# uguryagmur/RealTimeObjectDetection

Hardware: AMD Instinct MI355X
Metric: frames/sec YOLOv3 608x608 bs=8 (Darknet.forward + write_results; 2 batches in flight, write_results_async on a second stream) (higher is better)
Workload: dtype f16x2-split (3 MFMA products, f32 accumulate); 1 GPU; YOLOv3 cfg 608x608 batch=8 per GPU, split-f16 MFMA conv + fused head + GPU NMS (BASELINE configs[2]); precision=f16s3, tiles=autotune (this run), parallelism=frame-shard x1, in_flight_batches=2, detections_last_step=1699, candidates_last_step=1914, f16_range_overflow=False

## Files before the change

realtimeobjectdetection_amd/csrc/conv_bandd_common.h:

```cpp
#pragma once
#include "conv_f16s3_common.h"

namespace rtod {

#ifdef RTOD_TIMELINE
constexpr int BD_EPI_BLOCKS = 2048;
static __device__ unsigned long long g_bandd_epi[BD_EPI_BLOCKS * 5];
#define BD_ESTAMP(slot) { const unsigned long long tn_ = __builtin_amdgcn_s_memtime(); et_[slot] += tn_ - eprev_; eprev_ = tn_; }
#else
#define BD_ESTAMP(slot)
#endif

template <int NBASE, int PER = 2> __device__ __forceinline__ void bandd_wait_vmcnt_plus(int n) {
    static_assert(((NBASE == 4 || NBASE == 8) && PER == 2) || ((NBASE == 2 || NBASE == 4) && PER == 1), "two B sets of 1, 2 or 4 loads");
    asm volatile("" : "+s"(n));
    if (n == 0) vmcnt<NBASE>();
    else if (n == 1) vmcnt<NBASE + PER>();
    else if (n == 2) vmcnt<NBASE + 2 * PER>();
    else if (n == 3) vmcnt<NBASE + 3 * PER>();
    else if (n == 4) vmcnt<NBASE + 4 * PER>();
    else vmcnt<NBASE + 5 * PER>();
}

template <int BM, int BN, int WM, int WN, int NT, int RG, bool RES, int KG, bool F16 = false, bool RAW = false>
__device__ __forceinline__ void bandd_epilogue(const ConvArgs& a, f32x4 (&acc)[WM / 16][WN / 16], unsigned char* smem, int bm, int bn, int tid,
                                               int wm, int wn, int lr, int lh, int M, int kg) {
    constexpr int TM = WM / 16, TN = WN / 16, MT = 16, TS = BN;
    static_assert(BM % RG == 0 && RG % 16 == 0, "epilogue pass");
    static_assert(!RAW || (!RES && !F16), "raw-sum instances: no shortcut, no plain-f16 store");
#ifdef RTOD_TIMELINE
    unsigned long long et_[5] = {0, 0, 0, 0, 0};
    unsigned long long eprev_ = __builtin_amdgcn_s_memtime();
#endif
    float* T = reinterpret_cast<float*>(smem);
    float amax = 0.f;
    const float escale = RAW ? 1.0f : SPLIT_SCALE;
    constexpr int GPR = BN / 8;
// ... 91 lines not shown
```

realtimeobjectdetection_amd/csrc/conv_bandd_f16s3.hip:

```cpp
#include "conv_bandd_common.h"
#include <cstdio>
#include <cstdlib>
#include <map>
#include <vector>
#include <algorithm>

namespace rtod {

constexpr int BANDD_MAX_W = 94;
constexpr int BANDD_WIDE_W = 160;

#ifdef RTOD_TIMELINE
constexpr int BD_TL_BLOCKS = 2048, BD_TL_N = 8;
__device__ unsigned long long g_bandd_tl[BD_TL_BLOCKS * BD_TL_N];
#define BD_STAMP(slot) { const unsigned long long tn_ = __builtin_amdgcn_s_memtime(); tl_[slot] += tn_ - tl_prev_; tl_prev_ = tn_; }
#else
#define BD_STAMP(slot)
#endif
__host__ __device__ constexpr int bandd_rows(int bm, int w) { return (bm + 2 * w + 2 + 15) / 16 * 16; }

template <int BM, int BN, int NWM, int NWN, int MINW, int EPI, int BUFM, int KG, int MAXW>
__global__ __launch_bounds__(NWM * NWN * 64 * KG, MINW)
void conv_bandd_f16s3_kernel(const ConvArgs a, const int grid_m, const int grid_n) {
    constexpr bool F16 = epi_f16(EPI);
// ... 295 lines not shown
                    fprintf(stderr, "[timeline]   wg duration us min %.1f p10 %.1f p50 %.1f p90 %.1f max %.1f | end us p10 %.1f p50 %.1f p90 %.1f max %.1f | CUs seen %d, with 1/2/3/4/5 wgs: %d %d %d %d %d\n",
                            dur[0], dur[nb / 10], dur[nb / 2], dur[nb * 9 / 10], dur[nb - 1], en[nb / 10], en[nb / 2], en[nb * 9 / 10], en[nb - 1],
                            (int)per_cu.size(), hist[1], hist[2], hist[3], hist[4], hist[5]);
                    double ss[16] = {0}, sd[16] = {0}; int sn[16] = {0};
                    for (int b = 0; b < nb; ++b) { const int tg = (int)((h[b * BD_TL_N + 2] >> 16) & 15); ++sn[tg]; ss[tg] += (h[b * BD_TL_N] - t0) / 100.0; sd[tg] += (h[b * BD_TL_N + 1] - h[b * BD_TL_N]) / 100.0; }
                    for (int tg = 0; tg < 16; ++tg) if (sn[tg]) fprintf(stderr, "[timeline]   slot %d: %d wgs, mean start %.1f us, mean duration %.1f us\n", tg, sn[tg], ss[tg] / sn[tg], sd[tg] / sn[tg]);
                }
                ++printed;
            }
        }
    }
#endif
    return hip_fail(hipGetLastError(), "conv_bandd_f16s3 launch");
}

#define RTOD_BANDD_TILES(X) \
    X(0, 128, 128, 1, 4, 3, 0, 1, 94, "") X(1, 128, 128, 1, 4, 3, 1, 1, 94, ",db") X(2, 64, 128, 1, 4, 4, 1, 1, 94, ",db") \
    X(3, 64, 128, 1, 4, 4, 1, 2, 94, ",db,k2") X(4, 128, 128, 1, 4, 2, 1, 2, 94, ",db,k2") \
    X(5, 96, 128, 1, 4, 3, 1, 1, 94, ",db") X(6, 96, 128, 1, 4, 3, 1, 2, 94, ",db,k2") \
    X(7, 128, 128, 1, 4, 2, 0, 1, 160, ",w160") X(8, 48, 128, 1, 4, 3, 1, 2, 94, ",db,k2")

#define RTOD_X_INFO(idx, bm, bn, nwm, nwn, minw, db, kg, maxw, sfx) {bm, bn, "conv_bandd_f16s3<" #bm "x" #bn "," #nwm "x" #nwn sfx ">"},
static const ConvVariantInfo kBanddModes[BANDD_MODES] = { RTOD_BANDD_TILES(RTOD_X_INFO) };
#undef RTOD_X_INFO
const ConvVariantInfo& conv_bandd_mode_info(int idx) { return kBanddModes[idx < 0 || idx >= BANDD_MODES ? 0 : idx]; }
bool conv_bandd_wide_supported(int ksize, int stride, int pad, int cin, int w_in) {
    return ksize == 3 && stride == 1 && pad == 1 && cin % 32 == 0 && w_in > BANDD_MAX_W && w_in <= BANDD_WIDE_W;
}
int conv_bandd_mode_kg(int idx) {
#define RTOD_X_KG(i, bm, bn, nwm, nwn, minw, db, kg, maxw, sfx) if (idx == i) return kg;
// ... 31 lines not shown
```

realtimeobjectdetection_amd/csrc/plan.h:

```cpp
#pragma once
#include <functional>
#include <map>
#include <string>
#include <vector>

#include "rtod_internal.h"

namespace rtod {

enum LayerType { LT_CONV = 0, LT_SHORTCUT, LT_ROUTE, LT_UPSAMPLE, LT_MAXPOOL, LT_YOLO };
const char* layer_type_name(int t);

struct Layer {
    int index = 0;
    int type = LT_CONV;
    int cin = 0, cout = 0, hin = 0, win = 0, hout = 0, wout = 0;
    int size = 0, stride = 1, pad = 0;
    bool bn = false;
    int act = 0;
    bool nearest = false;
    bool decode_v5 = false;
    int pool_pad = 0;
    std::vector<int> srcs;
    std::vector<std::pair<int, int>> anchors;
// ... 92 lines not shown
    bool opt_patch_kernel = true;
    bool opt_ring_kernel = true;
    bool opt_pwd_kernel = true;
    bool opt_fuse_shortcut = true;
    bool opt_fuse_decode = true;
    bool opt_zero_copy_concat = true;
    bool opt_narrow_cin = false;
    bool opt_stem_pool = false;
    bool opt_keep_head_inputs = false;
    bool opt_keep_block_inputs = false;
    bool opt_keep_neck_activations = false;
    bool opt_keep_backbone_activations = false;
    bool opt_fuse_stem_pool = true;
    int opt_force_f16s3_variant = -1;
    int opt_force_f32_variant = -1;
    int32_t* overflow_flag = nullptr;
    std::vector<hipEvent_t> events;

    ~Plan();
    int parse(const std::string& cfg_text);
    int resolve_shapes();
    int plan_buffers();
    DecodeArgs decode_args(const Layer& yolo) const;
    int replan_or(const std::function<void()>& restore);
    void assign_arena();
    void layout_weights();
    bool uses_split(const Layer& L) const;
    int check_split_supported(int mode) const;
    int pack_weights(const float* w, size_t n, std::vector<float>& packed) const;
    void pack_conv(const PackedConv& pc, const float* p, float* blk) const;
// ... 80 lines not shown
```

realtimeobjectdetection_amd/csrc/plan_build.cpp:

```cpp
#include "plan.h"

#include <algorithm>
#include <cstdarg>
#include <sstream>

namespace rtod {

static thread_local std::string g_err;

void set_error(const char* fmt, ...) {
    char buf[1024];
    va_list ap;
    va_start(ap, fmt);
    vsnprintf(buf, sizeof(buf), fmt, ap);
    va_end(ap);
    g_err = buf;
}
const std::string& last_error_string() { return g_err; }

int hip_fail(hipError_t e, const char* what) {
    if (e == hipSuccess) return RTOD_OK;
    set_error("HIP error %d (%s) at %s", (int)e, hipGetErrorString(e), what);
    return RTOD_E_HIP;
}
// ... 32 lines not shown
        {"fuse_pointwise", &Plan::opt_fuse_pointwise}, {"ring_kernel", &Plan::opt_ring_kernel}, {"pwd_kernel", &Plan::opt_pwd_kernel},
        {"stem2_kernel", &Plan::opt_stem2_kernel}, {"k_slices", &Plan::opt_k_slices}, {"bn_batch_stats", &Plan::opt_bn_batch_stats},
        {"bn_batch_split", &Plan::opt_bn_batch_split}, {"bn_split_narrow", &Plan::opt_bn_split_narrow}, {"fuse_bn_pool", &Plan::opt_fuse_bn_pool},
        {"k_slice_workgroups", &Plan::opt_k_slice_workgroups}, {"k_slices_split", &Plan::opt_k_slices_split}, {"patch_kernel", &Plan::opt_patch_kernel},
        {"stem_kernel", &Plan::opt_stem_kernel}, {"band_kernel", &Plan::opt_band_kernel}, {"fuse_shortcut", &Plan::opt_fuse_shortcut},
        {"fuse_decode", &Plan::opt_fuse_decode}, {"zero_copy_concat", &Plan::opt_zero_copy_concat}, {"narrow_cin", &Plan::opt_narrow_cin},
        {"stem_pool", &Plan::opt_stem_pool}, {"fuse_stem_pool", &Plan::opt_fuse_stem_pool}, {"keep_head_inputs", &Plan::opt_keep_head_inputs},
        {"keep_block_inputs", &Plan::opt_keep_block_inputs}, {"keep_neck_activations", &Plan::opt_keep_neck_activations},
        {"keep_backbone_activations", &Plan::opt_keep_backbone_activations},
    };
    const std::string k(name);
    bool* flag = nullptr; int* num = nullptr;
    for (const auto& f : kFlags) if (k == f.name) flag = &(this->*f.flag);
    if (k == "force_f16s3_variant") num = &opt_force_f16s3_variant;
    else if (k == "force_f32_variant") num = &opt_force_f32_variant;
    else if (!flag) { set_error("set_option: unknown option '%s'", name); return RTOD_E_ARG; }
    if (flag == &opt_bn_batch_stats && value && height != width) { set_error("set_option: bn_batch_stats is not supported on a rectangular plan (%dx%d)", height, width); return RTOD_E_ARG; }
    const bool old_flag = flag ? *flag : false; const int old_num = num ? *num : 0;
    if (flag) *flag = value != 0; else *num = value;
    return replan_or([&] { if (flag) *flag = old_flag; else *num = old_num; });
}

int Plan::replan_or(const std::function<void()>& restore) {
    reset_planning();
    int rc = plan_buffers();
    if (!rc && precision >= 1) rc = check_split_supported(precision);
    if (rc) {
        const std::string msg = last_error_string();
        restore();
        reset_planning();
// ... 459 lines not shown
```

realtimeobjectdetection_amd/csrc/plan_forward.cpp:

```cpp
#include "plan.h"

#include <algorithm>
#include <cstring>

namespace rtod {

bool Plan::pw_active() const { return precision == 1 && opt_fuse_pointwise && !bn_split_active(); }
bool Plan::stem2_active() const { return precision == 1 && !bn_split_active() && opt_stem2_kernel && stem2_pattern && !keep_all && convs[launches[0].conv_slot].split; }
bool Plan::fusions_held() const { return opt_keep_backbone_activations; }
int Plan::fused_pool(int layer) const {
    if (keep_all) return -1;
    if (layer == 0 && precision >= 1 && stem_pool_pattern && convs[launches[0].conv_slot].stem16) return 1;
    return bn_narrow_active() && opt_fuse_bn_pool ? layers[layer].bn_pool : -1;
}

LaunchForm Plan::form(size_t li) const {
    LaunchForm f;
    const Launch& l = launches[li];
    switch (l.kind) {
        case LK_MAXPOOL:
            if (li > 0 && launches[li - 1].conv_slot >= 0 && fused_pool(launches[li - 1].layer) == l.layer) f.inside = (int)li - 1;
            return f;
        case LK_STEM: if (stem2_active()) f.inside = 1; break;
        case LK_CONV:
// ... 24 lines not shown
    const View in = view_of(l.in_layer);
    a.in = in.base; a.in_ldc = in.ldc; a.in_coff = in.coff;
    a.B = batch; a.Hi = L.hin; a.Wi = L.win; a.Cin = pc.cin_p;
    a.w = d_weights + pc.w_off; a.bias = d_weights + pc.b_off; a.K = pc.K; a.Kpad = pc.Kpad; a.Npad = pc.Npad;
    a.in_bytes = (unsigned)std::min<int64_t>((int64_t)batch * in.H * in.W * in.ldc * 4, 0xFFFFFFFFll);
    a.w_bytes = (unsigned)std::min<int64_t>((int64_t)pc.Npad * pc.Kpad * 2, 0xFFFFFFFFll);
    if (pc.split) {
        a.w_hi = reinterpret_cast<const _Float16*>(d_weights + pc.w_off);
        a.w_lo = reinterpret_cast<const _Float16*>(d_weights + pc.wl_off);
        a.inv_scale = d_weights + pc.s_off;
        a.f16 = precision == 2 ? 1 : 0;
    }
    a.kh = a.kw = L.size; a.stride = L.stride; a.pad = L.pad;
    a.Ho = L.hout; a.Wo = L.wout; a.Cout = L.cout; a.leaky = L.act;
    a.ovf = overflow_flag;
    if (in.C != pc.cin_p || in.H != L.hin || in.W != L.win) { set_error("forward: layer %d input view mismatch", l.layer); return RTOD_E_STATE; }
    if (l.out_layer == -2) { a.out = out; a.dec = l.dec; a.dec.train = train_decode; }
    else {
        const View o = view_of(l.out_layer);
        if (!o.base || o.C != L.cout || o.H != L.hout || o.W != L.wout) { set_error("forward: layer %d output view mismatch", l.layer); return RTOD_E_STATE; }
        a.out = o.base; a.out_ldc = o.ldc; a.out_coff = o.coff; a.out_split = o.split;
    }
    if (l.in2_layer >= 0) {
        const View r = view_of(l.in2_layer);
        if (!r.base || r.C != L.cout || r.H != L.hout || r.W != L.wout) { set_error("forward: layer %d residual view mismatch", l.layer); return RTOD_E_STATE; }
        a.res = r.base; a.res_ldc = r.ldc; a.res_coff = r.coff;
    }
    if (f.guest >= 0) {
        const Launch& g = launches[f.guest];
        const Layer& G = layers[g.layer];
// ... 215 lines not shown
```

realtimeobjectdetection_amd/csrc/plan_tiles.cpp:

```cpp
#include "plan.h"

#include <algorithm>
#include <mutex>

namespace rtod {

int Plan::choose_variant(const Layer& L, int batch) const {
    if (opt_force_f32_variant >= 0 && opt_force_f32_variant < CV_COUNT) return opt_force_f32_variant;
    if (L.cout <= 32) return CV_128x32;
    if (L.cout <= 64) return CV_128x64;
    const int64_t M = (int64_t)batch * L.hout * L.wout;
    const int64_t big = ((M + 127) / 128) * ((L.cout + 127) / 128);
    return big >= 512 ? CV_128x128 : CV_64x64;
}

int Plan::f32_slice_mode(const Launch& l, int batch, int variant) const {
    const PackedConv& pc = convs[l.conv_slot];
    if (pc.split || pc.stem || pc.slice_chunks <= 0) return 0;
    const Layer& L = layers[l.layer];
    const ConvVariantInfo& vi = conv_variant_info(variant);
    const int64_t M = (int64_t)batch * L.hout * L.wout;
    const int64_t tiles = ((M + vi.bm - 1) / vi.bm) * ((L.cout + vi.bn - 1) / vi.bn);
    const int64_t S = (pc.Kpad / 32 + pc.slice_chunks - 1) / pc.slice_chunks;
    return (opt_k_slice_workgroups && d_scratch && tiles < 512 && S * M * pc.Npad <= scratch_floats) ? 2 : 1;
}

bool Plan::tile_legal(const Launch& l, int v) const {
    const TileRef t = family_of(v);
    if (!t || l.kind != LK_CONV || l.conv_slot < 0 || !convs[l.conv_slot].split) return false;
    const PackedConv& pc = convs[l.conv_slot];
    const Layer& L = layers[l.layer];
    if (precision == 2 && !t.f16()) return false;
    if (raw_launch(l) && !t.raw()) return false;
    if (pc.narrow || t.is(TF_C16)) return pc.narrow && t.is(TF_C16);
    if (pc.ks_chunks > 0 || t.is(TF_KS)) return pc.ks_chunks > 0 && t.is(TF_KS);
    if (pc.band) return t.is(TF_BAND) && conv_band_mode_valid(t.mode, L.cin, L.hin, L.win);
    const bool hosts_pw = form(&l - &launches[0]).guest >= 0, plain = l.out_layer != -2 && !hosts_pw, same_map = L.hout == L.hin && L.wout == L.win;
    switch (t.fam->id) {
        case TF_GENERIC: return !(hosts_pw && t.fam->info(t.mode).bn < L.cout);
        case TF_BAND: return t.bandd_wide() && opt_band_kernel && plain && same_map && pc.Npad % 128 == 0 && pc.K == pc.Kpad &&
                             conv_bandd_wide_supported(L.size, L.stride, L.pad, pc.cin_p, L.win);
        case TF_RING: return !hosts_pw && L.act <= 1;
        case TF_PWD: return opt_pwd_kernel && plain && same_map && conv_pwd_supported(L.size, L.stride, L.pad, pc.cin_p);
        case TF_PATCH: return plain && L.act <= 1 && L.hout == L.hin && conv_patch_supported(L.size, L.stride, L.pad, L.cin, L.cout) &&
                              conv_patch_mode_valid(t.mode, L.cin, L.cout);
    }
    return false;
}

int Plan::default_tile(const Launch& l, int batch) const {
    const PackedConv& pc = convs[l.conv_slot];
// ... 13 lines not shown
}

int Plan::variant_for(const Launch& l, int batch) const {
    int want = opt_force_f16s3_variant;
    if (want < 0) {
        auto it = tuned.find(batch);
        const size_t idx = &l - &launches[0];
        if (it != tuned.end() && idx < it->second.size()) want = it->second[idx];
    }
    int v = want >= 0 && tile_legal(l, want) ? want : default_tile(l, batch);
    if (family_of(v).ks_sched_b() && !(opt_k_slice_workgroups && ks_sched_b_fits(l, batch))) --v;
    return v;
}

std::vector<int> Plan::tile_candidates(const Launch& l, int batch) const {
    static const int kOrder[TF_COUNT] = {TF_GENERIC, TF_PATCH, TF_BAND, TF_PWD, TF_RING, TF_C16, TF_KS};
    const int cout = layers[l.layer].cout;
    const bool ks_b = opt_k_slice_workgroups && ks_sched_b_fits(l, batch);
    std::vector<int> cand;
    for (int f : kOrder) {
        if ((f == TF_RING && !opt_ring_kernel) || (f == TF_PATCH && !opt_patch_kernel)) continue;
        const TileFamily& F = tile_family(f);
        for (int m = 0; m < F.modes; ++m) {
            const int bn = F.info(m).bn;
            const bool too_wide = f == TF_GENERIC || f == TF_RING ? bn > 64 && bn > 2 * ((cout + 63) / 64 * 64)
                                : f == TF_PATCH ? bn > 64 && bn > cout
                                : f == TF_PWD ? bn > 128 && bn > (cout + 127) / 128 * 128 : false;
            if (too_wide || (family_of(F.base + m).ks_sched_b() && !ks_b) || !tile_legal(l, F.base + m)) continue;
            cand.push_back(F.base + m);
        }
    }
// ... 1 lines not shown
}

int Plan::launch_split_variant(ConvArgs& a, const PackedConv& pc, int v, hipStream_t s) const {
    const TileRef t = family_of(v);
    if (!t) { set_error("variant %d is no split-f16 tile", v); return RTOD_E_STATE; }
    if (precision == 2 && !t.f16()) { set_error("variant %d has no plain-f16 instance", v); return RTOD_E_STATE; }
    if (a.raw_out && !t.raw()) { set_error("variant %d has no raw-sum instance", v); return RTOD_E_STATE; }
    if (pc.narrow != t.is(TF_C16)) {
        set_error(pc.narrow ? "variant %d requested for a narrow (Cin = 16) layer" : "narrow variant %d requested for a layer without tap-major weights", v);
        return RTOD_E_STATE;
    }
    if ((pc.ks_chunks > 0) != t.is(TF_KS)) {
        set_error(pc.ks_chunks > 0 ? "variant %d requested for a K-sliced layer" : "K-sliced variant %d requested for a layer that is not sliced", v);
        return RTOD_E_STATE;
    }
    if (pc.band != t.is(TF_BAND) && !(t.bandd_wide() && !pc.band)) {
        set_error(pc.band ? "variant %d requested for a band layer" : "band variant %d requested for a layer without band weights", v);
        return RTOD_E_STATE;
    }
    if (t.is(TF_KS)) {
        a.slice_chunks = pc.ks_chunks;
        a.partial = nullptr; a.partial_floats = 0;
        if (t.ks_sched_b()) { a.partial = d_scratch; a.partial_floats = scratch_floats; }
    }
    return t.fam->launch(a, t.mode, s);
}

static std::mutex g_tune_mutex;
static std::map<std::vector<int>, int> g_tune_memo;

int Plan::tune_launch(size_t li, ConvArgs& a, int batch, hipStream_t s) {
// ... 87 lines not shown
```

realtimeobjectdetection_amd/csrc/rtod_internal.h:

```cpp
#pragma once
#include <hip/hip_runtime.h>
#if defined(RTOD_STAMPS) && !defined(RTOD_DIAG)
#define RTOD_DIAG 1
#endif
#include <algorithm>
#include <atomic>
#include <cstdint>
#include <cstdio>
#include <string>
#include <vector>

#include "../../include/rtod.h"

namespace rtod {

void set_error(const char* fmt, ...);
int hip_fail(hipError_t e, const char* what);

#define RTOD_HIP(expr)                                              \
    do {                                                            \
        hipError_t _e = (expr);                                     \
        if (_e != hipSuccess) return ::rtod::hip_fail(_e, #expr);   \
    } while (0)

// ... 59 lines not shown
    int xcd_by_n = 0;
    int out_split = 0;
    int f16 = 0;
    float* raw_out = nullptr;
    int raw_ld = 0;
    int slice_chunks = 0;
    float* partial = nullptr;
    int64_t partial_floats = 0;
    const _Float16* pw_wh = nullptr;
    const _Float16* pw_wl = nullptr;
    const float* pw_inv_scale = nullptr;
    const float* pw_bias = nullptr;
    float* pw_out = nullptr;    int64_t pw_out_ldc = 0; int pw_out_coff = 0;
    int pw_npad = 0;
    int pw_cout = 0, pw_k = 0, pw_leaky = 0;
};

constexpr float SPLIT_SCALE = 8.0f;
constexpr float ACT_SCALE_F16S3 = SPLIT_SCALE;
constexpr float F16_MAX = 65504.0f;

#ifdef __HIPCC__
__device__ __forceinline__ void split_f16(float v, _Float16& h, _Float16& l, float& amax) {
    amax = fmaxf(amax, fabsf(v));
    const float vc = __builtin_amdgcn_fmed3f(v, -F16_MAX, F16_MAX);
    h = (_Float16)vc;
    l = (_Float16)(vc - (float)h);
}
__device__ __forceinline__ _Float16 f16_sat(float v, float& amax) {
    amax = fmaxf(amax, fabsf(v));
// ... 78 lines not shown
constexpr bool conv_c16_supported(int cin) { return cin == 16; }
const ConvVariantInfo& conv_c16_mode_info(int mode);
int conv_c16_default_mode(int cout, int64_t m);
int conv_c16_kernel_name(int mode, int epi, char* buf, size_t len);
int launch_conv_c16_f16s3(const ConvArgs& a, int mode, hipStream_t s);

constexpr int KS_TILES = 3;
constexpr int KS_MODES = 2 * KS_TILES;
constexpr int KS_VARIANT_BASE = 150;
constexpr int64_t KS_SCRATCH_FLOATS = 8ll << 20;
const ConvVariantInfo& conv_ks_mode_info(int mode);
int conv_ks_slices(const ConvArgs& a);
int conv_ks_kernel_name(int mode, int epi, char* buf, size_t len);
int launch_conv_ks_f16s3(const ConvArgs& a, int mode, hipStream_t s);

enum TileFamilyId { TF_GENERIC = 0, TF_BAND, TF_RING, TF_PWD, TF_PATCH, TF_C16, TF_KS, TF_COUNT };
struct TileFamily {
    int id, base, modes;
    int f16_from;
    int raw_from;
    const ConvVariantInfo& (*info)(int mode);
    int (*kernel_name)(int mode, int epi, char* buf, size_t len);
    int (*launch)(const ConvArgs& a, int mode, hipStream_t s);
};
struct TileRef {
    const TileFamily* fam; int mode;
    explicit operator bool() const { return fam != nullptr; }
    bool is(int family) const { return fam && fam->id == family; }
    bool f16() const { return fam && mode >= fam->f16_from; }
    bool raw() const { return fam && mode >= fam->raw_from; }
    bool ks_sched_b() const { return is(TF_KS) && (mode & 1); }
// ... 95 lines not shown
```

realtimeobjectdetection_amd/csrc/split_tiles.cpp:

```cpp
#include "rtod_internal.h"

namespace rtod {

static const TileFamily kFamilies[TF_COUNT] = {
    {TF_GENERIC, 0, HV_COUNT, 0, 0, conv_f16s3_variant_info, conv_f16s3_kernel_name, launch_conv_f16s3},
    {TF_BAND, BAND_VARIANT_BASE, BAND_MODES, BAND_LDS_MODES, BAND_LDS_MODES, conv_band_mode_info, conv_band_kernel_name, launch_conv_band_f16s3},
    {TF_RING, RING_VARIANT_BASE, RING_MODES, RING_MODES, RING_MODES, conv_ring_mode_info, conv_ring_kernel_name, launch_conv_ring_f16s3},
    {TF_PWD, PWD_VARIANT_BASE, PWD_MODES, 0, 0, conv_pwd_mode_info, conv_pwd_kernel_name, launch_conv_pwd_f16s3},
    {TF_PATCH, PATCH_VARIANT_BASE, PATCH_MODES, PATCH_MODES, PATCH_MODES, conv_patch_mode_info, conv_patch_kernel_name, launch_conv_patch_f16s3},
    {TF_C16, C16_VARIANT_BASE, C16_MODES, 0, 0, conv_c16_mode_info, conv_c16_kernel_name, launch_conv_c16_f16s3},
    {TF_KS, KS_VARIANT_BASE, KS_MODES, 0, KS_MODES, conv_ks_mode_info, conv_ks_kernel_name, launch_conv_ks_f16s3},
};
static_assert(HV_COUNT <= BAND_VARIANT_BASE, "generic tile ids end where the band family's begin");
static_assert(BAND_VARIANT_BASE + BAND_MODES <= RING_VARIANT_BASE, "band tile ids end where the ring family's begin");
static_assert(RING_VARIANT_BASE + RING_MODES <= PWD_VARIANT_BASE, "ring tile ids end where the pwd family's begin");
static_assert(PWD_VARIANT_BASE + PWD_MODES <= PATCH_VARIANT_BASE, "pwd tile ids end where the patch family's begin");
static_assert(PATCH_VARIANT_BASE + PATCH_MODES <= STEM2_VARIANT && STEM2_VARIANT < C16_VARIANT_BASE, "the fused stem's reported id lies between the patch and narrow families");
static_assert(C16_VARIANT_BASE + C16_MODES <= KS_VARIANT_BASE, "narrow tile ids end where the K-sliced family's begin");

TileRef family_of(int v) {
    for (const TileFamily& f : kFamilies)
        if (v >= f.base && v < f.base + f.modes) return {&f, v - f.base};
    return {nullptr, 0};
}

const TileFamily& tile_family(int family) { return kFamilies[family]; }

}
```

Measured before the change: 2632 frames/s.

## Add persistent band conv kernel overlapping tile epilogue with next tile's MFMA

Adds a new persistent-workgroup band conv family (TF_BANDP) in which each workgroup loops over several output tiles. The previous tile's epilogue (bias/activation, split store, shortcut add) is sliced into per-row pieces interleaved with the next tile's MFMA units, using a small per-wave LDS patch and buffer loads and stores. The aim is to hide the epilogue and launch tail behind compute. The family is added to the tile registry, but the candidate order list does not include TF_BANDP, so it runs only if forced or chosen elsewhere. It also adds a band_persist_slots option.

```diff
diff --git a/realtimeobjectdetection_amd/csrc/conv_bandd_common.h b/realtimeobjectdetection_amd/csrc/conv_bandd_common.h
--- a/realtimeobjectdetection_amd/csrc/conv_bandd_common.h
+++ b/realtimeobjectdetection_amd/csrc/conv_bandd_common.h
@@ -12,7 +12,7 @@
 #endif
 
 template <int NBASE, int PER = 2> __device__ __forceinline__ void bandd_wait_vmcnt_plus(int n) {
-    static_assert(((NBASE == 4 || NBASE == 8) && PER == 2) || ((NBASE == 2 || NBASE == 4) && PER == 1), "two B sets of 1, 2 or 4 loads");
+    static_assert(NBASE >= 2 && (PER == 1 || PER == 2) && NBASE + 5 * PER <= 63, "vmcnt range");
     asm volatile("" : "+s"(n));
     if (n == 0) vmcnt<NBASE>();
     else if (n == 1) vmcnt<NBASE + PER>();
@@ -21,6 +21,20 @@
     else if (n == 4) vmcnt<NBASE + 4 * PER>();
     else vmcnt<NBASE + 5 * PER>();
 }
+
+template <int I0, int N, typename F> __device__ __forceinline__ void static_for(F&& f) {
+    if constexpr (I0 < N) { f(std::integral_constant<int, I0>{}); static_for<I0 + 1, N>(f); }
+}
+__device__ __forceinline__ float buffer_load_f32(const __amdgpu_buffer_rsrc_t rsrc, unsigned voffset) {
+    float v;
+    asm volatile("buffer_load_dword %0, %1, %2, 0 offen" : "=v"(v) : "v"(voffset), "s"(rsrc) : "memory");
+    return v;
+}
+__device__ __forceinline__ void buffer_store_act16(const __amdgpu_buffer_rsrc_t rsrc, unsigned voffset, unsigned soffset, const f16x8& v) {
+    asm volatile("buffer_store_dwordx4 %0, %1, %2, %3 offen sc1\n\ts_nop 1" :: "v"(v), "v"(voffset), "s"(rsrc), "s"(soffset) : "memory");
+}
+constexpr int BP_PATCH_LD = 36;
+constexpr int BP_PATCH_BYTES = 16 * BP_PATCH_LD * 4;
 
 template <int BM, int BN, int WM, int WN, int NT, int RG, bool RES, int KG, bool F16 = false, bool RAW = false>
 __device__ __forceinline__ void bandd_epilogue(const ConvArgs& a, f32x4 (&acc)[WM / 16][WN / 16], unsigned char* smem, int bm, int bn, int tid,
diff --git a/realtimeobjectdetection_amd/csrc/conv_bandd_f16s3.hip b/realtimeobjectdetection_amd/csrc/conv_bandd_f16s3.hip
--- a/realtimeobjectdetection_amd/csrc/conv_bandd_f16s3.hip
+++ b/realtimeobjectdetection_amd/csrc/conv_bandd_f16s3.hip
@@ -333,6 +333,404 @@
     return hip_fail(hipGetLastError(), "conv_bandd_f16s3 launch");
 }
 
+template <int BM, int BN, int NWN, int EPI, int MAXW>
+__global__ __launch_bounds__(NWN * 64, 2)
+void conv_bandd_persist_kernel(const ConvArgs a, const int grid_m, const int grid_n) {
+    constexpr bool RES = epi_kind(EPI) == EPI_SPLIT_RES;
+    static_assert(!epi_f16(EPI) && !epi_raw(EPI), "f16s3 instances only");
+    constexpr int NW = NWN, WN = BN / NWN, TM = BM / 16, TN = WN / 16;
+    static_assert(BM % 16 == 0 && TN == 2 && TM >= 1 && TM <= 6, "strips of 32 columns; one piece per step, steps 7 and 8 free");
+    constexpr int NB = 2 * TN, PER = 2, UNITS = 9 * TM;
+    constexpr int NBLK_MAX = bandd_rows(BM, MAXW) / 16;
+    constexpr int PPW = (NBLK_MAX + NW - 1) / NW;
+    static_assert(PPW <= 5, "bandd_wait_vmcnt_plus covers 5 pairs");
+    constexpr int LR = RES ? 2 : 0, NPAR = 2 * TN, NST = 2;
+    constexpr int SLICE_UNIT = TM > 1 ? 1 : 0;
+
+    extern __shared__ __attribute__((aligned(16))) unsigned char smem[];
+#ifdef RTOD_TIMELINE
+    const unsigned long long tl_start_ = __builtin_amdgcn_s_memrealtime();
+    unsigned long long tl_prev_ = __builtin_amdgcn_s_memtime();
+    unsigned long long tl_[5] = {0, 0, 0, 0, 0};
+#endif
+    const int W = a.Wi, H = a.Hi;
+    const int NBLK = bandd_rows(BM, W) / 16;
+    const int BUF = (NBLK + 1) * 2048;
+    const int zero_off = NBLK * 2048;
+    const int nt = grid_m * grid_n, slots = (int)gridDim.x;
+    const int wave = __builtin_amdgcn_readfirstlane((int)threadIdx.x >> 6), lane = (int)threadIdx.x & 63;
+    const int lr = lane & 15, lh = lane >> 4;
+    const int M = a.B * H * W;
+    const int NBv = BM + 2 * W + 2;
+    const unsigned PS = (unsigned)a.in_ldc * 4u;
+    const unsigned lo_plane = (unsigned)a.in_ldc * 2u;
+    float* const patch = reinterpret_cast<float*>(smem + 2 * BUF + wave * BP_PATCH_BYTES);
+
+    if (threadIdx.x < 16) {
+        const int b = threadIdx.x >> 3, k = threadIdx.x & 7;
+        *reinterpret_cast<u32x4*>(smem + b * BUF + zero_off + (k >> 2) * 1024 + (k & 3) * 16) = u32x4{0u, 0u, 0u, 0u};
+    }
+
+    const __amdgpu_buffer_rsrc_t rs_a = buffer_rsrc(a.in, a.in_bytes);
+    const __amdgpu_buffer_rsrc_t rs_wh = buffer_rsrc(a.w_hi, a.w_bytes);
+    const __amdgpu_buffer_rsrc_t rs_wl = buffer_rsrc(a.w_lo, a.w_bytes);
+    const unsigned lds0 = (unsigned)(size_t)smem;
+    const int n_dma = (NBLK + NW - 1) / NW;
+    auto dma_band = [&](int m0, int cc, int buf) __attribute__((always_inline)) {
+        const unsigned soff = (unsigned)cc * 64u;
+        const unsigned base = lds0 + (unsigned)(buf * BUF);
+        int l = (int)threadIdx.x;
+        asm volatile("" : "+v"(l));
+        const int dma_lrow = (l & 63) >> 2;
+        const unsigned dma_cpart = (unsigned)(a.in_coff + ((l & 3) ^ ((dma_lrow >> 1) & 3)) * 8) * 2u;
+        const int r0 = wave * 16 + dma_lrow;
+#pragma unroll
+        for (int k = 0; k < PPW; ++k) {
+            const int blk = wave + k * NW;
+            const int r = r0 + k * NW * 16;
+            const int q = m0 - W - 1 + r;
+            const unsigned vo = (blk < NBLK && r < NBv && (unsigned)q < (unsigned)M) ? (unsigned)q * PS + dma_cpart : OOB;
+            const unsigned dst = base + (unsigned)(blk < NBLK ? blk * 2048 : zero_off);
+            if (k < n_dma) lds_dma_pair<0x400>(rs_a, vo, soff, lo_plane + soff, dst);
+        }
+    };
+    auto tile_bid = [&](int id) __attribute__((always_inline)) { return a.xcd_by_n ? id : xcd_remap(id, nt); };
+
+    const unsigned wchunk = (unsigned)a.Npad * (HBK * 2);
+    const int n_cc = a.Cin / 32;
+    auto bvoff_of = [&](int id) __attribute__((always_inline)) -> unsigned {
+        if (id >= nt) return OOB;
+        const int bid = tile_bid(id);
+        const int n0 = (bid % grid_n) * BN + wave * WN;
+        return n0 + lr < a.Npad ? (unsigned)((n0 + lr) * 32 + lh * 8) * 2u : OOB;
+    };
+    u32x4 Bq[3][TN][2];
+    int ld_tile = (int)blockIdx.x, ld_cc = 0;
+    unsigned ld_koff = 0u, ld_bvoff = bvoff_of(ld_tile);
+    auto load_b = [&](u32x4 (&q)[TN][2], int tap) __attribute__((always_inline)) {
+        const unsigned koff = ld_koff + (unsigned)tap * wchunk;
+        q[0][0] = buffer_load_b128(rs_wh, ld_bvoff, koff);
+        q[0][1] = buffer_load_b128(rs_wl, ld_bvoff, koff);
+        q[1][0] = buffer_load_b128<1024>(rs_wh, ld_bvoff, koff);
+        q[1][1] = buffer_load_b128<1024>(rs_wl, ld_bvoff, koff);
+        if (tap == 8) {
+            if (++ld_cc == n_cc) { ld_cc = 0; ld_koff = 0u; ld_tile += slots; ld_bvoff = bvoff_of(ld_tile); }
+            else ld_koff += 9u * wchunk;
+        }
+    };
+
+    constexpr int NVM = (TM + 2) / 3;
+    unsigned vmw[NVM];
+    auto set_masks = [&](int m0) __attribute__((always_inline)) {
+#pragma unroll
+        for (int w = 0; w < NVM; ++w) vmw[w] = 0u;
+        const int hw = H * W;
+        int m = m0 + lr;
+        const int mm = m < M ? m : 0;
+        int b = mm / hw;
+        int r = mm - b * hw;
+        int oy = r / W, ox = r - oy * W;
+#pragma unroll
+        for (int i = 0; i < TM; ++i) {
+            unsigned vm = 0;
+            if (m < M) {
+                const unsigned xm = (ox >= 1 ? 1u : 0u) | 2u | (ox + 1 < W ? 4u : 0u);
+                vm = (oy >= 1 ? xm : 0u) | (xm << 3) | (oy + 1 < H ? xm << 6 : 0u);
+            }
+            vmw[i / 3] |= vm << ((i % 3) * 9);
+            m += 16; ox += 16;
+            if (W >= 16) {
+                const bool wx = ox >= W; ox = wx ? ox - W : ox; oy += wx ? 1 : 0;
+                const bool wy = oy >= H; oy = wy ? oy - H : oy;
+            } else {
+                while (ox >= W) { ox -= W; ++oy; }
+                while (oy >= H) { oy -= H; ++b; }
+            }
+        }
+    };
+
+    f32x4 acc[TM][TN], eacc[TM][TN];
+#pragma unroll
+    for (int i = 0; i < TM; ++i)
+#pragma unroll
+        for (int j = 0; j < TN; ++j)
+#pragma unroll
+            for (int e = 0; e < 4; ++e) acc[i][j][e] = 0.f;
+
+    const int lh4 = lh << 4;
+    f16x8 Ah[3], Al[3];
+    typedef const f16x8 __attribute__((address_space(3))) lds_f16x8;
+    int prow_c = lr;
+    auto read_unit = [&](int t, int i, int bufoff, f16x8& h, f16x8& l) __attribute__((always_inline)) {
+        const int row = prow_c + (t / 3) * W + (t % 3);
+        const int x0 = (((row & ~15) << 7) | ((row & 15) << 6) | (((row << 3) ^ lh4) & 0x30)) + bufoff;
+        const int sel = __builtin_amdgcn_sbfe((int)vmw[i / 3], (i % 3) * 9 + t, 1);
+        const int z = bufoff + zero_off - 2048 * i;
+        int o;
+        asm("v_bfi_b32 %0, %1, %2, %3" : "=v"(o) : "v"(sel), "v"(x0), "s"(z));
+        h = *reinterpret_cast<lds_f16x8*>((unsigned)(o + 2048 * i));
+        l = *reinterpret_cast<lds_f16x8*>((unsigned)(o + 2048 * i + 1024));
+    };
+
+    const __amdgpu_buffer_rsrc_t rs_bias = buffer_rsrc(a.bias, (unsigned)a.Cout * 4u);
+    const __amdgpu_buffer_rsrc_t rs_inv = buffer_rsrc(a.inv_scale, (unsigned)a.Cout * 4u);
+    const __amdgpu_buffer_rsrc_t rs_out = buffer_rsrc(a.out, OOB);
+    const __amdgpu_buffer_rsrc_t rs_res = buffer_rsrc(RES ? a.res : a.out, OOB);
+    int elane = lane;
+    const unsigned out_px = (unsigned)a.out_ldc * 4u, res_px = (unsigned)a.res_ldc * 4u;
+    int e_m0 = 0, e_n0 = 0;
+    float par_b[TN], par_i[TN], amax = 0.f;
+    u32x4 rq_h, rq_l;
+    auto issue_params = [&]() __attribute__((always_inline)) {
+#pragma unroll
+        for (int j = 0; j < TN; ++j) {
+            const unsigned vo = (unsigned)(e_n0 + j * 16 + (elane & 15)) * 4u;
+            par_b[j] = buffer_load_f32(rs_bias, vo);
+            par_i[j] = buffer_load_f32(rs_inv, vo);
+        }
+    };
+    auto piece_m = [&](int p) __attribute__((always_inline)) { return e_m0 + p * 16 + (elane >> 2); };
+    auto issue_res = [&](int p) __attribute__((always_inline)) {
+        const int m = piece_m(p), ec8 = (elane & 3) * 8;
+        const unsigned vo = (m < M && e_n0 + ec8 < a.Cout) ? (unsigned)m * res_px + (unsigned)(a.res_coff + e_n0 + ec8) * 2u : OOB;
+        rq_h = buffer_load_b128(rs_res, vo, 0u);
+        rq_l = buffer_load_b128(rs_res, vo, (unsigned)a.res_ldc * 2u);
+    };
+    auto piece = [&](auto P_, auto WAIT_) __attribute__((always_inline)) {
+        constexpr int p = decltype(P_)::value, WAIT = decltype(WAIT_)::value;
+        const int erow = elane >> 2, ec8 = (elane & 3) * 8, elr = elane & 15, elh = elane >> 4;
+        if constexpr (p == 0 || RES) {
+            vmcnt<WAIT>();
+            if constexpr (p == 0) { tie(par_b); tie(par_i); }
+            if constexpr (RES) tie(rq_h, rq_l);
+            __builtin_amdgcn_sched_barrier(0);
+        }
+        epi_by_activation(a.leaky, [&](auto act) {
+#pragma unroll
+            for (int j = 0; j < TN; ++j) {
+                const float bias = par_b[j] * SPLIT_SCALE, inv = par_i[j] * SPLIT_SCALE;
+#pragma unroll
+                for (int e = 0; e < 4; ++e)
+                    patch[(e + 4 * elh) * BP_PATCH_LD + j * 16 + elr] = epi_scale_act1<decltype(act)::value>(eacc[p][j][e], inv, bias, 1.0f / SPLIT_SCALE);
+            }
+        });
+        __builtin_amdgcn_wave_barrier();
+        const f32x4 v0 = *reinterpret_cast<const f32x4*>(patch + erow * BP_PATCH_LD + ec8);
+        const f32x4 v1 = *reinterpret_cast<const f32x4*>(patch + erow * BP_PATCH_LD + ec8 + 4);
+        __builtin_amdgcn_wave_barrier();
+        float v[8] = {v0[0], v0[1], v0[2], v0[3], v1[0], v1[1], v1[2], v1[3]};
+        if constexpr (RES) {
+            const f16x8 qh = __builtin_bit_cast(f16x8, rq_h), ql = __builtin_bit_cast(f16x8, rq_l);
+#pragma unroll
+            for (int e = 0; e < 8; ++e) v[e] += (float)qh[e] + (float)ql[e];
+        }
+        f16x8 ph, pl;
+#pragma unroll
+        for (int e = 0; e < 8; ++e) { _Float16 h, l; split_f16(v[e], h, l, amax); ph[e] = h; pl[e] = l; }
+        if constexpr (RES && p + 1 < TM) issue_res(p + 1);
+        const int m = piece_m(p);
+        const unsigned vo = (m < M && e_n0 + ec8 < a.Cout) ? (unsigned)m * out_px + (unsigned)(a.out_coff + e_n0 + ec8) * 2u : OOB;
+        buffer_store_act16(rs_out, vo, 0u, ph);
+        buffer_store_act16(rs_out, vo, (unsigned)a.out_ldc * 2u, pl);
+    };
+
+    auto chunk_body = [&](int ep, int bufoff, int dma_behind) __attribute__((always_inline)) {
+        asm volatile("" : "+s"(ep));
+        read_unit(0, 0, bufoff, Ah[0], Al[0]);
+        if constexpr (UNITS > 1) read_unit(1 / TM, 1 % TM, bufoff, Ah[1], Al[1]);
+        __builtin_amdgcn_sched_barrier(0);
+        static_for<0, UNITS>([&](auto U_) __attribute__((always_inline)) {
+            constexpr int u = decltype(U_)::value, t = u / TM, i = u % TM;
+            constexpr auto ops = [](int s) { return s < 0 || s > TM ? 0 : s == 0 ? NPAR + LR : NST + (s < TM ? LR : 0); };
+            if constexpr (i == 0) {
+                load_b(Bq[(t + 2) % 3], (t + 2) % 9);
+                constexpr int X = t >= 2 ? ops(t - 2) + ops(t - 1) : t == 1 ? ops(0) : 0;
+                if constexpr (t >= 2) {
+                    if constexpr (X > 0) { if (ep) vmcnt<2 * NB + X>(); else vmcnt<2 * NB>(); }
+                    else vmcnt<2 * NB>();
+                } else if constexpr (X > 0) {
+                    if (ep) bandd_wait_vmcnt_plus<2 * NB + X, PER>(dma_behind); else bandd_wait_vmcnt_plus<2 * NB, PER>(dma_behind);
+                } else bandd_wait_vmcnt_plus<2 * NB, PER>(dma_behind);
+                tie_bset<false>(Bq[t % 3]);
+                __builtin_amdgcn_sched_barrier(0);
+            }
+            if constexpr (u + 2 < UNITS) read_unit((u + 2) / TM, (u + 2) % TM, bufoff, Ah[(u + 2) % 3], Al[(u + 2) % 3]);
+            const f16x8 ah = Ah[u % 3], al = Al[u % 3];
+#pragma unroll
+            for (int j = 0; j < TN; ++j) {
+                const f16x8 bh = __builtin_bit_cast(f16x8, Bq[t % 3][j][0]);
+                const f16x8 bl = __builtin_bit_cast(f16x8, Bq[t % 3][j][1]);
+                acc[i][j] = __builtin_amdgcn_mfma_f32_16x16x32_f16(al, bh, acc[i][j], 0, 0, 0);
+                acc[i][j] = __builtin_amdgcn_mfma_f32_16x16x32_f16(ah, bl, acc[i][j], 0, 0, 0);
+                acc[i][j] = __builtin_amdgcn_mfma_f32_16x16x32_f16(ah, bh, acc[i][j], 0, 0, 0);
+            }
+            if constexpr (i == SLICE_UNIT && t <= TM) {
+                __builtin_amdgcn_sched_barrier(0);
+                if (ep) {
+                    if constexpr (t == 0) { issue_params(); if constexpr (RES) issue_res(0); }
+                    else piece(std::integral_constant<int, (t >= 1 ? t - 1 : 0)>{}, std::integral_constant<int, NB + (t >= 2 ? NST : 0)>{});
+                }
+            }
+            __builtin_amdgcn_sched_barrier(0);
+        });
+    };
+
+    int tile = (int)blockIdx.x;
+    int bid = tile_bid(tile);
+    int m0 = (bid / grid_n) * BM;
+    dma_band(m0, 0, 0);
+    load_b(Bq[0], 0);
+    load_b(Bq[1], 1);
+    vmcnt<0>();
+    tie_bset<false>(Bq[0]); tie_bset<false>(Bq[1]);
+    __builtin_amdgcn_sched_barrier(0);
+    __syncthreads();
+    BD_STAMP(0)
+    __builtin_amdgcn_s_setprio(2);
+    int g = 0;
+    bool pending = false;
+#pragma unroll 1
+    for (;;) {
+        set_masks(m0);
+        const int next = tile + slots;
+        const bool has_next = next < nt;
+        const int next_bid = has_next ? tile_bid(next) : 0;
+        const int next_m0 = (next_bid / grid_n) * BM;
+#pragma unroll 1
+        for (int cc = 0; cc < n_cc; ++cc, ++g) {
+            const int buf = g & 1;
+            const int bufoff = (int)lds0 + buf * BUF;
+            asm volatile("" : "+v"(prow_c));
+            asm volatile("" : "+v"(elane));
+#pragma unroll
+            for (int w = 0; w < NVM; ++w) asm volatile("" : "+v"(vmw[w]));
+            __builtin_amdgcn_sched_barrier(0);
+            __builtin_amdgcn_s_barrier();
+            int dma_behind = 0;
+            if (cc + 1 < n_cc) { dma_band(m0, cc + 1, buf ^ 1); dma_behind = n_dma; }
+            else if (has_next) { dma_band(next_m0, 0, buf ^ 1); dma_behind = n_dma; }
+            BD_STAMP(1)
+            const int ep = __builtin_amdgcn_readfirstlane(pending && cc == 0 ? 1 : 0);
+            chunk_body(ep, bufoff, dma_behind);
+            pending = pending && !ep;
+#ifdef RTOD_TIMELINE
+            if (ep) BD_STAMP(3) else BD_STAMP(2)
+#endif
+        }
+        e_m0 = m0; e_n0 = (bid % grid_n) * BN + wave * WN;
+#pragma unroll
+        for (int i = 0; i < TM; ++i)
+#pragma unroll
+            for (int j = 0; j < TN; ++j) {
+                eacc[i][j] = acc[i][j];
+#pragma unroll
+                for (int e = 0; e < 4; ++e) acc[i][j][e] = 0.f;
+            }
+        pending = true;
+        if (!has_next) break;
+        tile = next; bid = next_bid; m0 = next_m0;
+    }
+    vmcnt<0>();
+    tie_bset<false>(Bq[0]); tie_bset<false>(Bq[1]); tie_bset<false>(Bq[2]);
+    __builtin_amdgcn_sched_barrier(0);
+    __builtin_amdgcn_s_setprio(0);
+    BD_STAMP(1)
+    issue_params();
+    if constexpr (RES) issue_res(0);
+    static_for<0, TM>([&](auto P_) __attribute__((always_inline)) {
+        piece(P_, std::integral_constant<int, (decltype(P_)::value >= 1 ? NST : 0)>{});
+    });
+    split_overflow_report(a.ovf, amax);
+#ifdef RTOD_TIMELINE
+    BD_STAMP(4)
+    if (threadIdx.x == 0 && blockIdx.x < BD_TL_BLOCKS) {
+        unsigned long long* o = g_bandd_tl + blockIdx.x * BD_TL_N;
+        o[0] = tl_start_; o[1] = __builtin_amdgcn_s_memrealtime();
+        o[2] = 0;
+        for (int i = 0; i < 5; ++i) o[3 + i] = tl_[i];
+    }
+#endif
+}
+
+template <int BM, int MAXW>
+static int launch_bandp(const ConvArgs& a, hipStream_t s) {
+    constexpr int BN = 128, NWN = 4;
+    const int M = a.B * a.Ho * a.Wo;
+    const int gm = (M + BM - 1) / BM, gn = (a.Cout + BN - 1) / BN, nt = gm * gn;
+    if (a.Cin % 32) { set_error("launch_conv_bandp: Cin=%d not a multiple of 32", a.Cin); return RTOD_E_ARG; }
+    if ((int64_t)M * a.out_ldc * 4 >= (int64_t)OOB || (a.res && (int64_t)M * a.res_ldc * 4 >= (int64_t)OOB)) {
+        set_error("launch_conv_bandp: output or shortcut view of 2 GiB or more"); return RTOD_E_ARG;
+    }
+    ConvArgs ax = a;
+    ax.xcd_by_n = (gn % 8 == 0 && (int64_t)a.Cout * a.K > (int64_t)M * a.Cin) ? 1 : 0;
+    const int lds = 2 * (bandd_rows(BM, a.Wi) / 16 + 1) * 2048 + NWN * BP_PATCH_BYTES;
+    if (lds > 160 * 1024) { set_error("launch_conv_bandp: %d bytes of LDS", lds); return RTOD_E_ARG; }
+    int cus = device_cu_count();
+    if (cus <= 0) cus = 256;
+    int grid = std::min(nt, cus * (2 * lds <= 160 * 1024 ? 2 : 1));
+    if (a.persist_slots > 0) grid = std::min(grid, a.persist_slots);
+    auto k_res = conv_bandd_persist_kernel<BM, BN, NWN, EPI_SPLIT_RES, MAXW>;
+    auto k_plain = conv_bandd_persist_kernel<BM, BN, NWN, EPI_SPLIT, MAXW>;
+    static std::atomic<unsigned long long> attr_done{0};
+    const int mx = std::min(2 * (bandd_rows(BM, MAXW) / 16 + 1) * 2048 + NWN * BP_PATCH_BYTES, 160 * 1024);
+    if (int rc = lds_opt_in(attr_done, mx, "conv_bandd_persist", k_res, k_plain)) return rc;
+    if (a.res) hipLaunchKernelGGL(k_res, dim3(grid), dim3(NWN * 64), lds, s, ax, gm, gn);
+    else hipLaunchKernelGGL(k_plain, dim3(grid), dim3(NWN * 64), lds, s, ax, gm, gn);
+#ifdef RTOD_TIMELINE
+    {
+        static int printed = 0;
+        const int nb = grid < BD_TL_BLOCKS ? grid : BD_TL_BLOCKS;
+        if (printed < 200 && hipDeviceSynchronize() == hipSuccess) {
+            static unsigned long long h[BD_TL_BLOCKS * BD_TL_N];
+            if (hipMemcpyFromSymbol(h, HIP_SYMBOL(g_bandd_tl), sizeof(unsigned long long) * BD_TL_N * nb) == hipSuccess) {
+                unsigned long long t0 = ~0ull, t1 = 0;
+                double ph[5] = {0, 0, 0, 0, 0}, rt = 0;
+                for (int b = 0; b < nb; ++b) { if (h[b * BD_TL_N] < t0) t0 = h[b * BD_TL_N]; if (h[b * BD_TL_N + 1] > t1) t1 = h[b * BD_TL_N + 1]; }
+                for (int b = 0; b < nb; ++b) {
+                    for (int i = 0; i < 5; ++i) ph[i] += (double)h[b * BD_TL_N + 3 + i];
+                    rt += (double)(h[b * BD_TL_N + 1] - h[b * BD_TL_N]);
+                }
+                fprintf(stderr, "[timeline] bandd_persist<%d,%d> W=%d Cin=%d Cout=%d res=%d tiles=%d wgs=%d lds=%d | span %.1f us | wg mean %.1f us | kcycles/wg: own prologue %.1f tops %.1f plain bodies %.1f overlapped bodies %.1f final drain %.1f\n",
+                        BM, BN, a.Wi, a.Cin, a.Cout, a.res ? 1 : 0, nt, grid, lds, (t1 - t0) / 100.0, rt / nb / 100.0,
+                        ph[0] / nb / 1e3, ph[1] / nb / 1e3, ph[2] / nb / 1e3, ph[3] / nb / 1e3, ph[4] / nb / 1e3);
+                ++printed;
+            }
+        }
+    }
+#endif
+    return hip_fail(hipGetLastError(), "conv_bandd_persist launch");
+}
+
+#define RTOD_BANDP_TILES(X) X(0, 64, 94) X(1, 48, 94) X(2, 96, 94)
+#define RTOD_X_INFO(m, bm, maxw) {bm, 128, "conv_bandd_f16s3<" #bm "x128,1x4,persist>"},
+static const ConvVariantInfo kBandpModes[BANDP_MODES] = { RTOD_BANDP_TILES(RTOD_X_INFO) };
+#undef RTOD_X_INFO
+const ConvVariantInfo& conv_bandp_mode_info(int mode) { return kBandpModes[mode < 0 || mode >= BANDP_MODES ? 0 : mode]; }
+int conv_bandp_mode_kg(int mode) { return mode >= 0 && mode < BANDP_MODES ? 1 : 0; }
+int conv_bandp_kernel_name(int mode, int epi, char* buf, size_t len) {
+#define RTOD_X_NAME(m, bm, maxw) \
+    if (mode == m) return snprintf(buf, len, "void rtod::conv_bandd_persist_kernel<" #bm ", 128, 4, %d, " #maxw ">(rtod::ConvArgs, int, int)", epi);
+    RTOD_BANDP_TILES(RTOD_X_NAME)
+#undef RTOD_X_NAME
+    return -1;
+}
+int launch_conv_bandp_f16s3(const ConvArgs& a, int mode, hipStream_t s) {
+    if (int rc = check_split_conv_args(a, "launch_conv_bandp", false)) return rc;
+    if (a.kh != 3 || a.stride != 1 || a.pad != 1 || a.Cin % 32 || a.Wi > BANDD_MAX_W || a.kw != 3 || a.Ho != a.Hi || a.Wo != a.Wi || a.dec.enabled || a.pw_wh) {
+        set_error("launch_conv_bandp: unsupported shape (k=%d s=%d pad=%d Cin=%d W=%d)", a.kh, a.stride, a.pad, a.Cin, a.Wi); return RTOD_E_ARG;
+    }
+    if (a.in_ldc % 8 || a.in_coff % 8 || a.K != a.Kpad || a.K != 9 * a.Cin || a.Npad % 128) { set_error("launch_conv_bandp: bad view / K"); return RTOD_E_ARG; }
+    if (a.raw_out || a.f16) { set_error("launch_conv_bandp: f16s3 instances only"); return RTOD_E_ARG; }
+    if (a.out_coff % 2 || (a.res && a.res_coff % 2)) { set_error("launch_conv_bandp: output / shortcut view not dword aligned"); return RTOD_E_ARG; }
+    switch (mode) {
+#define RTOD_X_CASE(m, bm, maxw) case m: return launch_bandp<bm, maxw>(a, s);
+        RTOD_BANDP_TILES(RTOD_X_CASE)
+#undef RTOD_X_CASE
+    }
+    set_error("launch_conv_bandp: mode %d unsupported", mode);
+    return RTOD_E_ARG;
+}
+
 #define RTOD_BANDD_TILES(X) \
     X(0, 128, 128, 1, 4, 3, 0, 1, 94, "") X(1, 128, 128, 1, 4, 3, 1, 1, 94, ",db") X(2, 64, 128, 1, 4, 4, 1, 1, 94, ",db") \
     X(3, 64, 128, 1, 4, 4, 1, 2, 94, ",db,k2") X(4, 128, 128, 1, 4, 2, 1, 2, 94, ",db,k2") \
diff --git a/realtimeobjectdetection_amd/csrc/plan.h b/realtimeobjectdetection_amd/csrc/plan.h
--- a/realtimeobjectdetection_amd/csrc/plan.h
+++ b/realtimeobjectdetection_amd/csrc/plan.h
@@ -130,6 +130,7 @@
     bool opt_fuse_stem_pool = true;
     int opt_force_f16s3_variant = -1;
     int opt_force_f32_variant = -1;
+    int opt_band_persist_slots = 0;
     int32_t* overflow_flag = nullptr;
     std::vector<hipEvent_t> events;
 
diff --git a/realtimeobjectdetection_amd/csrc/plan_build.cpp b/realtimeobjectdetection_amd/csrc/plan_build.cpp
--- a/realtimeobjectdetection_amd/csrc/plan_build.cpp
+++ b/realtimeobjectdetection_amd/csrc/plan_build.cpp
@@ -70,6 +70,7 @@
     for (const auto& f : kFlags) if (k == f.name) flag = &(this->*f.flag);
     if (k == "force_f16s3_variant") num = &opt_force_f16s3_variant;
     else if (k == "force_f32_variant") num = &opt_force_f32_variant;
+    else if (k == "band_persist_slots") { if (value < 0) { set_error("set_option: band_persist_slots=%d", value); return RTOD_E_ARG; } num = &opt_band_persist_slots; }
     else if (!flag) { set_error("set_option: unknown option '%s'", name); return RTOD_E_ARG; }
     if (flag == &opt_bn_batch_stats && value && height != width) { set_error("set_option: bn_batch_stats is not supported on a rectangular plan (%dx%d)", height, width); return RTOD_E_ARG; }
     const bool old_flag = flag ? *flag : false; const int old_num = num ? *num : 0;
diff --git a/realtimeobjectdetection_amd/csrc/plan_forward.cpp b/realtimeobjectdetection_amd/csrc/plan_forward.cpp
--- a/realtimeobjectdetection_amd/csrc/plan_forward.cpp
+++ b/realtimeobjectdetection_amd/csrc/plan_forward.cpp
@@ -62,6 +62,7 @@
     a.kh = a.kw = L.size; a.stride = L.stride; a.pad = L.pad;
     a.Ho = L.hout; a.Wo = L.wout; a.Cout = L.cout; a.leaky = L.act;
     a.ovf = overflow_flag;
+    a.persist_slots = opt_band_persist_slots;
     if (in.C != pc.cin_p || in.H != L.hin || in.W != L.win) { set_error("forward: layer %d input view mismatch", l.layer); return RTOD_E_STATE; }
     if (l.out_layer == -2) { a.out = out; a.dec = l.dec; a.dec.train = train_decode; }
     else {
diff --git a/realtimeobjectdetection_amd/csrc/plan_tiles.cpp b/realtimeobjectdetection_amd/csrc/plan_tiles.cpp
--- a/realtimeobjectdetection_amd/csrc/plan_tiles.cpp
+++ b/realtimeobjectdetection_amd/csrc/plan_tiles.cpp
@@ -34,7 +34,11 @@
     if (raw_launch(l) && !t.raw()) return false;
     if (pc.narrow || t.is(TF_C16)) return pc.narrow && t.is(TF_C16);
     if (pc.ks_chunks > 0 || t.is(TF_KS)) return pc.ks_chunks > 0 && t.is(TF_KS);
-    if (pc.band) return t.is(TF_BAND) && conv_band_mode_valid(t.mode, L.cin, L.hin, L.win);
+    if (pc.band) {
+        if (t.is(TF_BANDP)) return pc.Npad % 128 == 0 && conv_bandp_mode_kg(t.mode) == conv_band_layer_kg(L.cin, L.hin, L.win);
+        return t.is(TF_BAND) && conv_band_mode_valid(t.mode, L.cin, L.hin, L.win);
+    }
+    if (t.is(TF_BANDP)) return false;
     const bool hosts_pw = form(&l - &launches[0]).guest >= 0, plain = l.out_layer != -2 && !hosts_pw, same_map = L.hout == L.hin && L.wout == L.win;
     switch (t.fam->id) {
         case TF_GENERIC: return !(hosts_pw && t.fam->info(t.mode).bn < L.cout);
@@ -78,7 +82,7 @@
 }
 
 std::vector<int> Plan::tile_candidates(const Launch& l, int batch) const {
-    static const int kOrder[TF_COUNT] = {TF_GENERIC, TF_PATCH, TF_BAND, TF_PWD, TF_RING, TF_C16, TF_KS};
+    static const int kOrder[] = {TF_GENERIC, TF_PATCH, TF_BAND, TF_PWD, TF_RING, TF_C16, TF_KS};
     const int cout = layers[l.layer].cout;
     const bool ks_b = opt_k_slice_workgroups && ks_sched_b_fits(l, batch);
     std::vector<int> cand;
@@ -110,7 +114,7 @@
         set_error(pc.ks_chunks > 0 ? "variant %d requested for a K-sliced layer" : "K-sliced variant %d requested for a layer that is not sliced", v);
         return RTOD_E_STATE;
     }
-    if (pc.band != t.is(TF_BAND) && !(t.bandd_wide() && !pc.band)) {
+    if (pc.band != (t.is(TF_BAND) || t.is(TF_BANDP)) && !(t.bandd_wide() && !pc.band)) {
         set_error(pc.band ? "variant %d requested for a band layer" : "band variant %d requested for a layer without band weights", v);
         return RTOD_E_STATE;
     }
diff --git a/realtimeobjectdetection_amd/csrc/rtod_internal.h b/realtimeobjectdetection_amd/csrc/rtod_internal.h
--- a/realtimeobjectdetection_amd/csrc/rtod_internal.h
+++ b/realtimeobjectdetection_amd/csrc/rtod_internal.h
@@ -97,6 +97,7 @@
     float* pw_out = nullptr;    int64_t pw_out_ldc = 0; int pw_out_coff = 0;
     int pw_npad = 0;
     int pw_cout = 0, pw_k = 0, pw_leaky = 0;
+    int persist_slots = 0;
 };
 
 constexpr float SPLIT_SCALE = 8.0f;
@@ -205,7 +206,14 @@
 int conv_ks_kernel_name(int mode, int epi, char* buf, size_t len);
 int launch_conv_ks_f16s3(const ConvArgs& a, int mode, hipStream_t s);
 
-enum TileFamilyId { TF_GENERIC = 0, TF_BAND, TF_RING, TF_PWD, TF_PATCH, TF_C16, TF_KS, TF_COUNT };
+constexpr int BANDP_MODES = 3;
+constexpr int BANDP_VARIANT_BASE = 170;
+const ConvVariantInfo& conv_bandp_mode_info(int mode);
+int conv_bandp_mode_kg(int mode);
+int conv_bandp_kernel_name(int mode, int epi, char* buf, size_t len);
+int launch_conv_bandp_f16s3(const ConvArgs& a, int mode, hipStream_t s);
+
+enum TileFamilyId { TF_GENERIC = 0, TF_BAND, TF_RING, TF_PWD, TF_PATCH, TF_C16, TF_KS, TF_BANDP, TF_COUNT };
 struct TileFamily {
     int id, base, modes;
     int f16_from;
diff --git a/realtimeobjectdetection_amd/csrc/split_tiles.cpp b/realtimeobjectdetection_amd/csrc/split_tiles.cpp
--- a/realtimeobjectdetection_amd/csrc/split_tiles.cpp
+++ b/realtimeobjectdetection_amd/csrc/split_tiles.cpp
@@ -10,6 +10,7 @@
     {TF_PATCH, PATCH_VARIANT_BASE, PATCH_MODES, PATCH_MODES, PATCH_MODES, conv_patch_mode_info, conv_patch_kernel_name, launch_conv_patch_f16s3},
     {TF_C16, C16_VARIANT_BASE, C16_MODES, 0, 0, conv_c16_mode_info, conv_c16_kernel_name, launch_conv_c16_f16s3},
     {TF_KS, KS_VARIANT_BASE, KS_MODES, 0, KS_MODES, conv_ks_mode_info, conv_ks_kernel_name, launch_conv_ks_f16s3},
+    {TF_BANDP, BANDP_VARIANT_BASE, BANDP_MODES, BANDP_MODES, BANDP_MODES, conv_bandp_mode_info, conv_bandp_kernel_name, launch_conv_bandp_f16s3},
 };
 static_assert(HV_COUNT <= BAND_VARIANT_BASE, "generic tile ids end where the band family's begin");
 static_assert(BAND_VARIANT_BASE + BAND_MODES <= RING_VARIANT_BASE, "band tile ids end where the ring family's begin");
@@ -17,6 +18,7 @@
 static_assert(PWD_VARIANT_BASE + PWD_MODES <= PATCH_VARIANT_BASE, "pwd tile ids end where the patch family's begin");
 static_assert(PATCH_VARIANT_BASE + PATCH_MODES <= STEM2_VARIANT && STEM2_VARIANT < C16_VARIANT_BASE, "the fused stem's reported id lies between the patch and narrow families");
 static_assert(C16_VARIANT_BASE + C16_MODES <= KS_VARIANT_BASE, "narrow tile ids end where the K-sliced family's begin");
+static_assert(KS_VARIANT_BASE + KS_MODES <= BANDP_VARIANT_BASE, "K-sliced tile ids end where the persistent band tiles' begin");
 
 TileRef family_of(int v) {
     for (const TileFamily& f : kFamilies)
```

Result: slower. 2573 frames/s (-2.3%).
